# jhamrick/bayesian-quadrature

Hardware: NVIDIA B200
Metric: expected_Z_var candidate evals/sec (higher is better)
Workload: dtype f64

## Files before the change

bayesian_quadrature_b200/csrc/bq_score.cu:

```cuda
#include <cstdlib>

#include "bq_common.cuh"

namespace bqb {


constexpr int CHUNK_FRAGS_MAX = 256;
#ifndef BQB_REL_GK
#define BQB_REL_GK 4
#endif

__device__ __forceinline__ unsigned smem_u32(const void *p) { return (unsigned)__cvta_generic_to_shared(p); }
__device__ __forceinline__ void mbar_init(unsigned long long *bar, unsigned count) {
    asm volatile("mbarrier.init.shared::cta.b64 [%0], %1;" ::"r"(smem_u32(bar)), "r"(count) : "memory");
}
__device__ __forceinline__ void mbar_init_fence() { asm volatile("fence.mbarrier_init.release.cluster;" ::: "memory"); }
__device__ __forceinline__ void mbar_expect_tx(unsigned long long *bar, unsigned bytes) {
    asm volatile("mbarrier.arrive.expect_tx.shared::cta.b64 _, [%0], %1;" ::"r"(smem_u32(bar)), "r"(bytes) : "memory");
}
__device__ __forceinline__ void mbar_wait(unsigned long long *bar, unsigned parity) {
    asm volatile(
        "{\n"
        ".reg .pred p;\n"
        "MBAR_WAIT:\n"
        "mbarrier.try_wait.parity.shared::cta.b64 p, [%0], %1;\n"
        "@p bra MBAR_DONE;\n"
        "bra MBAR_WAIT;\n"
        "MBAR_DONE:\n"
        "}" ::"r"(smem_u32(bar)), "r"(parity) : "memory");
}
__device__ __forceinline__ void bulk_g2s(void *dst, const void *src, unsigned bytes, unsigned long long *bar) {
    asm volatile("cp.async.bulk.shared::cluster.global.mbarrier::complete_tx::bytes [%0], [%1], %2, [%3];" ::"r"(smem_u32(dst)),
                 "l"(src), "r"(bytes), "r"(smem_u32(bar)) : "memory");
}

constexpr int SCR_STRIDE = 40;
constexpr int SCR_DENSE = 4;

__device__ __forceinline__ void fetch_points(double *row, const double *__restrict__ xa, long long base, int na, int lane) {
    if (base + lane < na) {
        const unsigned d = (unsigned)__cvta_generic_to_shared(row + lane);
        asm volatile("cp.async.ca.shared.global [%0], [%1], 8;" ::"r"(d), "l"(xa + base + lane) : "memory");
    } else {
        row[lane] = 0.0;
    }
}

template <int KS, int NT, int WARPS, bool STREAM, int TABN>
struct ScoreSmem {
    static constexpr int NBC = KS / 2;
    static __host__ __device__ constexpr int operands(int ndb_max, int chunk_frags, int nb_res) {
        return STREAM ? 2 * chunk_frags * 32 + ndb_max * KS * 32 : 2 * tri_frags(nb_res) * 32 + ndb_max * 2 * nb_res * 32;
    }
    static __host__ __device__ constexpr int scr(int nrow) { return (SCR_DENSE + nrow) * SCR_STRIDE + 64; }
    static __host__ __device__ constexpr int doubles(int n_small, int ndb_max, int chunk_frags, int nb_res, int nrow) {
        return n_small + operands(ndb_max, chunk_frags, nb_res) + WARPS * scr(nrow);
    }
};

template <int THREADS>
__device__ __forceinline__ void stage(double *dst, const double *__restrict__ src, int count) {
    const double2 *s2 = reinterpret_cast<const double2 *>(src);
    double2 *d2 = reinterpret_cast<double2 *>(dst);
    for (int i = threadIdx.x; i < count / 2; i += THREADS) d2[i] = __ldg(s2 + i);
}

template <int KS> struct KMask { using type = unsigned; };
template <> struct KMask<40> { using type = unsigned long long; };
template <> struct KMask<64> { using type = unsigned long long; };

constexpr double CUT_ARG = 72.0;
static_assert(CUT_ARG == 72.0, "keep in step with ScoreArgs::cut_arg and include/bq_b200.h");

__device__ __forceinline__ int float_key(float f) {
    const int i = __float_as_int(f);
    return i >= 0 ? i : (i ^ 0x7fffffff);
}
__device__ __forceinline__ float key_float(int k) { return __int_as_float(k >= 0 ? k : (k ^ 0x7fffffff)); }

template <int KS>
__device__ __forceinline__ void gen_masks(double xv, bool valid, double cut_l, double cut_tl, int nsp, int lane,
                                          const double *s_xs, typename KMask<KS>::type &mask_l, typename KMask<KS>::type &mask_tl) {
    using mask_t = typename KMask<KS>::type;
    constexpr int NW = (KS + 7) / 8;
    const double xc = fmin(fmax(xv, -1e30), 1e30);
    const int klo = valid ? float_key(__double2float_rd(xc)) : 0x7fffffff;
    const int khi = valid ? float_key(__double2float_ru(xc)) : (int)0x80000000;
    const double xlo = (double)key_float(__reduce_min_sync(0xffffffffu, klo));
    const double xhi = (double)key_float(__reduce_max_sync(0xffffffffu, khi));
    if (!(xlo <= xhi)) { mask_l = 0; mask_tl = 0; return; }
    const double c = 0.5 * (xlo + xhi), hw = 0.5 * (xhi - xlo);
    double dk[NW];
    double dmin = INFINITY;
#pragma unroll
    for (int i = 0; i < NW; ++i) {
        const int k = 32 * i + lane;
        dk[i] = (k < nsp) ? fabs(s_xs[k] - c) : INFINITY;
        dmin = fmin(dmin, dk[i]);
    }
    const float dcf = __int_as_float(__reduce_min_sync(0xffffffffu, __float_as_int(__double2float_ru(fmin(dmin, 3e38)))));
    const double reach = (double)dcf + hw;
    const double r2_l = fma(reach, reach, cut_l), r2_tl = fma(reach, reach, cut_tl);
    mask_t ml = 0, mt = 0;
#pragma unroll
    for (int i = 0; i < NW; ++i) {
        const double t = fmax(dk[i] - hw, 0.0), t2 = t * t;
        const bool in = 32 * i + lane < nsp;
        unsigned bl = __ballot_sync(0xffffffffu, in && t2 <= r2_l), bt = __ballot_sync(0xffffffffu, in && t2 <= r2_tl);
        bl |= bl >> 1; bl |= bl >> 2; bl &= 0x11111111u;
        bl = (bl | (bl >> 3)) & 0x03030303u; bl = (bl | (bl >> 6)) & 0x000f000fu; bl = (bl | (bl >> 12)) & 0xffu;
        bt |= bt >> 1; bt |= bt >> 2; bt &= 0x11111111u;
        bt = (bt | (bt >> 3)) & 0x03030303u; bt = (bt | (bt >> 6)) & 0x000f000fu; bt = (bt | (bt >> 12)) & 0xffu;
        ml |= (mask_t)bl << (8 * i);
        mt |= (mask_t)bt << (8 * i);
    }
    mask_l = ml;
    mask_tl = mt;
}

template <int NT> __host__ __device__ constexpr int exp_group() { return NT == 1 ? 8 : 4; }
template <int KS, int NT, int TABN, bool TL, int GK = exp_group<NT>()>
__device__ __forceinline__ void gen_exps(double (&bf)[KS][NT], const double (&x)[NT], double C, int d2max_hi,
                                         typename KMask<KS>::type mask, int kq, const double *s_xs, const double *s_atl,
                                         const double *s_tab, double (&tm)[NT], int tol2_hi, int (&close)[NT], int nkv = KS) {
    using mask_t = typename KMask<KS>::type;
    int minhi[NT];
#pragma unroll
    for (int nt = 0; nt < NT; ++nt) minhi[nt] = 0x7fffffff;
#pragma unroll
    for (int g = 0; g < (KS + GK - 1) / GK; ++g) {
        if ((mask >> (GK * g)) & (((mask_t)1 << GK) - 1)) {
#pragma unroll
            for (int j = 0; j < GK; ++j) {
                const int ks = GK * g + j;
                if (ks < KS) {
                    const double xs = s_xs[4 * ks + kq];
#pragma unroll
                    for (int nt = 0; nt < NT; ++nt) {
                        const double d = x[nt] - xs;
                        const double d2 = d * d;
                        const double e = exp_kernel<TABN>(d2, C, d2max_hi, s_tab);
                        bf[ks][nt] = e;
                        if (TL) {
                            minhi[nt] = min(minhi[nt], __double2hiint(d2));
                            if (ks < nkv) tm[nt] = fma(s_atl[4 * ks + kq], e, tm[nt]);
                        }
                    }
                }
            }
        }
    }
    if (TL) {
#pragma unroll
        for (int nt = 0; nt < NT; ++nt) close[nt] = (minhi[nt] <= tol2_hi);
    }
}

__device__ __forceinline__ int isclose_exact(double x, const double *s_xs, const double *s_tol, int nsp, int kq) {
    int c = 0;
    for (int k = kq; k < nsp; k += 4) c |= (fabs(x - s_xs[k]) <= s_tol[k]);
    return c;
}

__device__ __forceinline__ void async_commit() { asm volatile("cp.async.commit_group;" ::: "memory"); }
template <int N> __device__ __forceinline__ void async_wait() { asm volatile("cp.async.wait_group %0;" ::"n"(N) : "memory"); }

template <int KS, int NT>
__device__ __forceinline__ void row_block_acc(const double *af, int lim, const double (&bf)[KS][NT], double (&c0)[NT],
                                              double (&c1)[NT], double (&e0)[NT], double (&e1)[NT],
                                              typename KMask<KS>::type mask) {
    using mask_t = typename KMask<KS>::type;
    constexpr bool DUAL = (NT == 1);
#pragma unroll
    for (int ks = 0; ks < KS; ks += 2) {
        if (ks >= lim) break;
        if (mask & ((mask_t)3 << ks)) {
            const double a0 = af[ks * 32], a1 = af[(ks + 1) * 32];
#pragma unroll
            for (int nt = 0; nt < NT; ++nt) {
                dmma(c0[nt], c1[nt], a0, bf[ks][nt]);
                if (DUAL) dmma(e0[nt], e1[nt], a1, bf[ks + 1][nt]);
                else dmma(c0[nt], c1[nt], a1, bf[ks + 1][nt]);
            }
        }
    }
}
template <int NT>
__device__ __forceinline__ void row_block_finish(const double (&c0)[NT], const double (&c1)[NT], const double (&e0)[NT],
                                                 const double (&e1)[NT], double (&q0)[NT], double (&q1)[NT]) {
    constexpr bool DUAL = (NT == 1);
#pragma unroll
    for (int nt = 0; nt < NT; ++nt) {
        const double r0 = DUAL ? c0[nt] + e0[nt] : c0[nt], r1 = DUAL ? c1[nt] + e1[nt] : c1[nt];
        q0[nt] = fma(r0, r0, q0[nt]);
        q1[nt] = fma(r1, r1, q1[nt]);
    }
}
template <int KS, int NT>
__device__ __forceinline__ void row_block(const double *af, int lim, const double (&bf)[KS][NT], double (&q0)[NT],
                                          double (&q1)[NT], typename KMask<KS>::type mask) {
    double c0[NT], c1[NT], e0[NT], e1[NT];
#pragma unroll
    for (int nt = 0; nt < NT; ++nt) { c0[nt] = c1[nt] = e0[nt] = e1[nt] = 0.0; }
    row_block_acc<KS, NT>(af, lim, bf, c0, c1, e0, e1, mask);
    row_block_finish<NT>(c0, c1, e0, e1, q0, q1);
}

template <int KS, int NT, int K0>
__device__ __forceinline__ void pair_group(const double *afA, const double *afB, int limA, const double (&bf)[KS][NT],
                                           double (&a0)[NT], double (&a1)[NT], double (&b0)[NT], double (&b1)[NT],
                                           double (&c0)[NT], double (&c1)[NT], double (&d0)[NT], double (&d1)[NT]) {
    constexpr int ks = K0;
    if (ks + 4 <= limA) {
        double fa[4], fb[4];
#pragma unroll
        for (int j = 0; j < 4; ++j) { fa[j] = afA[(ks + j) * 32]; fb[j] = afB[(ks + j) * 32]; }
#pragma unroll
        for (int j = 0; j < 4; j += 2)
#pragma unroll
            for (int nt = 0; nt < NT; ++nt) {
                dmma(a0[nt], a1[nt], fa[j], bf[ks + j][nt]);
                dmma(c0[nt], c1[nt], fb[j], bf[ks + j][nt]);
                dmma(b0[nt], b1[nt], fa[j + 1], bf[ks + j + 1][nt]);
                dmma(d0[nt], d1[nt], fb[j + 1], bf[ks + j + 1][nt]);
            }
    } else if (ks + 2 <= limA) {
        const double fa0 = afA[ks * 32], fa1 = afA[(ks + 1) * 32];
        double fb[4];
#pragma unroll
        for (int j = 0; j < 4; ++j) fb[j] = afB[(ks + j) * 32];
#pragma unroll
        for (int nt = 0; nt < NT; ++nt) {
            dmma(a0[nt], a1[nt], fa0, bf[ks][nt]);
            dmma(c0[nt], c1[nt], fb[0], bf[ks][nt]);
            dmma(b0[nt], b1[nt], fa1, bf[ks + 1][nt]);
            dmma(d0[nt], d1[nt], fb[1], bf[ks + 1][nt]);
            dmma(c0[nt], c1[nt], fb[2], bf[ks + 2][nt]);
            dmma(d0[nt], d1[nt], fb[3], bf[ks + 3][nt]);
        }
    } else {
        const double fb0 = afB[ks * 32], fb1 = afB[(ks + 1) * 32];
#pragma unroll
        for (int nt = 0; nt < NT; ++nt) {
            dmma(c0[nt], c1[nt], fb0, bf[ks][nt]);
            dmma(d0[nt], d1[nt], fb1, bf[ks + 1][nt]);
        }
    }
}

template <int KS, int NT, bool PLAIN = false>
__device__ __forceinline__ void row_block_pair(const double *afA, const double *afB, int limA, const double (&bf)[KS][NT],
                                               double (&q0)[NT], double (&q1)[NT], typename KMask<KS>::type mask, int g0, int kend) {
    using mask_t = typename KMask<KS>::type;
    static_assert(KS % 4 == 0 && KS <= 64, "k-steps come in groups of 4, at most 16 groups");
    double a0[NT], a1[NT], b0[NT], b1[NT], c0[NT], c1[NT], d0[NT], d1[NT];
#pragma unroll
    for (int nt = 0; nt < NT; ++nt) { a0[nt] = a1[nt] = b0[nt] = b1[nt] = c0[nt] = c1[nt] = d0[nt] = d1[nt] = 0.0; }
    const int kstop = min(kend, limA + 2);
#define BQB_GRP(G)                                                                                                       \
    case G:                                                                                                              \
        if constexpr (4 * (G) < KS) {                                                                                    \
            if (4 * (G) >= kstop) break;                                                                                 \
            if (mask & ((mask_t)15 << (4 * (G))))                            \
                pair_group<KS, NT, 4 * (G)>(afA, afB, limA, bf, a0, a1, b0, b1, c0, c1, d0, d1);                         \
        }                                                                                                                \
        [[fallthrough]];
#define BQB_GRP_PLAIN(G)                                                                                                 \
    if constexpr (4 * (G) < KS) {                                                                                        \
        if (4 * (G) < kstop) {                                                                                           \
            pair_group<KS, NT, 4 * (G)>(afA, afB, limA, bf, a0, a1, b0, b1, c0, c1, d0, d1);
// ... 187 lines not shown
__device__ __forceinline__ void tri_pass(const double *af_res, double (&bf)[KS][NT], double (&q0)[NT], double (&q1)[NT],
                                         int nb, int lane, typename KMask<KS>::type mask, int k0, const Wide<NT> &w) {
    using mask_t = typename KMask<KS>::type;
    static_assert(ROLLED || !REL, "the band-relative tile needs the rolled row-block loop");
    phase_sync<ALIGN>();
    if constexpr (ROLLED) {
        row_blocks_rolled<KS, NT, TABN, REL>(af_res + lane, 0, nb, bf, q0, q1, mask, k0, w);
    } else {
#pragma unroll
        for (int rb = 0; rb < KS / 2; ++rb) {
            constexpr int BITS = 8 * sizeof(mask_t);
            const mask_t low = (2 * rb + 2 >= BITS) ? ~(mask_t)0 : (((mask_t)1 << (2 * rb + 2)) - 1);
            if (rb < nb && (mask & low)) row_block<KS, NT>(af_res + tri_frags(rb) * 32 + lane, 2 * rb + 2, bf, q0, q1, mask);
        }
    }
}

struct SlabPlan {
    int klo, W, rb_first, R, nchunk;
};
template <int KS>
__device__ __forceinline__ SlabPlan make_slab_plan(typename KMask<KS>::type um, int nks, int nb, int cap_frags) {
    SlabPlan p;
    if (um == 0) { p.klo = p.W = p.rb_first = p.R = p.nchunk = 0; return p; }
    const unsigned long long m = um;
    const int lo = __ffsll((long long)m) - 1, hi = 64 - __clzll((long long)m);
    p.klo = lo & ~3;
    const int khi = min((hi + 3) & ~3, nks);
    p.W = khi - p.klo;
    p.rb_first = p.klo >> 1;
    p.R = max(2, (cap_frags / p.W) & ~1);
    p.nchunk = (nb - p.rb_first + p.R - 1) / p.R;
    return p;
}
struct Stream {
    unsigned long long *bar;
    double *buf;
    int stride;
    unsigned phase;
};
__device__ __forceinline__ void slab_issue(const double *__restrict__ op, const SlabPlan &p, int c, int nb, const Stream &st, int b,
                                           int lane) {
    const int rb0 = p.rb_first + c * p.R, n = min(nb - rb0, p.R);
    if (lane == 0) mbar_expect_tx(st.bar + b, (unsigned)(n * p.W * 256));
    __syncwarp();
    if (lane < n)
        bulk_g2s(st.buf + b * st.stride + lane * p.W * 32, op + (size_t)(tri_frags(rb0 + lane) + p.klo) * 32, (unsigned)(p.W * 256),
                 st.bar + b);
}
template <int KS, int NT, int TABN, bool REL>
__device__ __forceinline__ void slab_rows(const double *buf, const SlabPlan &p, int rb0, int rb1, double (&bf)[KS][NT],
                                          double (&q0)[NT], double (&q1)[NT], typename KMask<KS>::type mask, int lane, int k0,
                                          const Wide<NT> &w) {
    if constexpr (REL) {
        if (w.on) {
            const int kfirst = __ffsll((long long)w.mask) - 1;
#pragma unroll 1
            for (int rb = max(rb0, kfirst >> 1); rb < rb1; ++rb)
                wide_row_block<KS, NT, TABN>(buf + ((rb - rb0) * p.W - p.klo) * 32 + lane, 2 * rb + 2, w, bf, q0, q1);
            return;
        }
    }
    if (!mask) return;
    int g0, kend;
    mask_groups(mask, g0, kend);
    const int kfirst = k0 + __ffsll((long long)(unsigned long long)mask) - 1;
    int rb = rb0;
    const bool rect = REL && plain_band(mask, g0, kend);
    const int kend2 = (64 - __clzll((long long)(unsigned long long)mask) + 1) & ~1;
    const int rbf = rect ? min(rb1, max(rb0, ((k0 + kend2) >> 1) & ~1)) : rb1;
#pragma unroll 1
    for (; rb + 1 < rbf; rb += 2) {
        if (2 * rb + 4 <= kfirst) continue;
        const double *afA = buf + ((rb - rb0) * p.W - p.klo + k0) * 32 + lane;
        if (REL && rect) row_block_pair<KS, NT, REL>(afA, afA + p.W * 32, 2 * rb + 2 - k0, bf, q0, q1, mask, g0, kend);
        else row_block_pair<KS, NT>(afA, afA + p.W * 32, 2 * rb + 2 - k0, bf, q0, q1, mask, g0, kend);
    }
    if constexpr (REL) {
        if (rect && rb + 1 < rb1) {
            const int npair = (rb1 - rb) >> 1;
            rect_dispatch<KS, NT>(kend2 >> 1, buf + ((rb - rb0) * p.W - p.klo + k0) * 32 + lane, npair, p.W * 32, 2 * p.W * 32, 0, 0, bf, q0,
                                  q1);
            rb += 2 * npair;
        }
    }
    if (rb < rb1) row_block<KS, NT>(buf + ((rb - rb0) * p.W - p.klo + k0) * 32 + lane, 2 * rb + 2 - k0, bf, q0, q1, mask);
}
template <int KS, int NT, int TABN, bool REL>
__device__ __forceinline__ void slab_pass(const double *__restrict__ op, const SlabPlan &p, bool res, bool first_sub, Stream &st,
                                          double (&bf)[KS][NT], double (&q0)[NT], double (&q1)[NT], int nb, int lane, int warp,
                                          typename KMask<KS>::type mask, int k0, const Wide<NT> &w) {
    const int nch = res ? (p.nchunk ? 1 : 0) : p.nchunk;
    const int R = res ? nb - p.rb_first : p.R;
#pragma unroll 1
    for (int c = 0; c < nch; ++c) {
        const int b = res ? 0 : (c & 1);
        if (!res || first_sub) {
            mbar_wait(st.bar + b, (st.phase >> b) & 1u);
            st.phase ^= 1u << b;
        }
        const int rb0 = p.rb_first + c * R;
        slab_rows<KS, NT, TABN, REL>(st.buf + b * st.stride, p, rb0, min(nb, rb0 + R), bf, q0, q1, mask, lane, k0, w);
        if (!res) {
            __syncthreads();
            if (warp == 0 && c + 2 < nch) slab_issue(op, p, c + 2, nb, st, b, lane);
        }
    }
}

template <int KB, int NT, int GK = exp_group<NT>()>
__device__ __forceinline__ void dense_acc(const double *af, int nk, const double (&bf)[KB][NT], typename KMask<KB>::type mask,
                                          double (&c0)[NT], double (&c1)[NT], double (&e0)[NT], double (&e1)[NT]) {
    using mask_t = typename KMask<KB>::type;
#pragma unroll
    for (int g = 0; g < KB / GK; ++g) {
        if ((mask >> (GK * g)) & (((mask_t)1 << GK) - 1)) {
            double fa[GK];
#pragma unroll
            for (int j = 0; j < GK; ++j) fa[j] = (GK * g + j < nk) ? af[(GK * g + j) * 32] : 0.0;
#pragma unroll
            for (int j = 0; j < GK; j += 2)
#pragma unroll
                for (int nt = 0; nt < NT; ++nt) {
                    dmma(c0[nt], c1[nt], fa[j], bf[GK * g + j][nt]);
                    dmma(e0[nt], e1[nt], fa[j + 1], bf[GK * g + j + 1][nt]);
                }
        }
    }
}

template <int NT>
__device__ __forceinline__ void park_q(double (&q0)[NT], double (&q1)[NT], double *scr, int row, int col0, int kq, int pq) {
#pragma unroll
    for (int nt = 0; nt < NT; ++nt) {
#pragma unroll
        for (int o = 4; o < 32; o <<= 1) {
            q0[nt] += __shfl_xor_sync(0xffffffffu, q0[nt], o);
            q1[nt] += __shfl_xor_sync(0xffffffffu, q1[nt], o);
        }
        if (pq == 0) *reinterpret_cast<double2 *>(scr + row * SCR_STRIDE + col0 + nt * 8 + 2 * kq) = make_double2(q0[nt], q1[nt]);
    }
}

template <int KS, int NT, int WARPS, int MINB, bool STREAM, int TABN, int ALIGN, bool ROLLED, int BK, int MODE>
__global__ void __launch_bounds__(WARPS * 32, MINB) bq_score_kernel(ScoreArgs a) {
    constexpr bool EPI = MODE == 1, PRED = MODE == 2;
    constexpr bool REL = BK > 0;
    constexpr int KB = REL ? BK : KS;
    static_assert(!REL || (BK % 8 == 0 && BK <= KS), "band tile: whole exp groups, no larger than the class");
    using rmask_t = typename KMask<KB>::type;
    constexpr int GKK = REL ? BQB_REL_GK : exp_group<NT>();
    using SM = ScoreSmem<KS, NT, WARPS, STREAM, TABN>;
    constexpr bool LOCKSTEP = STREAM || ALIGN != 0;
    static_assert(ALIGN <= 1 || WARPS % ALIGN == 0, "barrier groups of whole warps");
    constexpr int THREADS = WARPS * 32;
    constexpr int SUB = 4 / NT;
    extern __shared__ __align__(16) double smem[];
    const Layout lay = a.lay;
    __shared__ __align__(16) double s_tab[TABN];
    double *s_small = smem;
    double *s_ops = s_small + lay.n_small;
    double *s_af_l = s_ops;
    constexpr bool RT_SIZES = KS > 16;
    const int nb_res = RT_SIZES ? a.nb_res : KS / 2, nrow_res = RT_SIZES ? a.nrow_res : 8 * a.ndb_max;
    double *s_af_d = STREAM ? s_ops + 2 * a.chunk_frags * 32 : s_af_l + tri_frags(nb_res) * 32;
    double *s_af_t = s_af_d + a.ndb_max * 2 * nb_res * 32;
    double *s_scr = s_ops + SM::operands(a.ndb_max, a.chunk_frags, nb_res);

    const int tid = threadIdx.x, lane = tid & 31, warp = tid >> 5;
    const int inst = a.inst0 + blockIdx.y;
    const double *M = a.models + (size_t)inst * lay.total;

    __shared__ int s_cta_st;
    if (tid == 0) s_cta_st = 0;
    for (int i = tid; i < TABN; i += THREADS) s_tab[i] = a.exp_tab[(TABN == 2048 ? 0 : 2048) + i];
    for (int i = tid; i < lay.n_small; i += THREADS) s_small[i] = M[i];
    __syncthreads();
    const int nc = (int)s_small[H_NC], nsp = (int)s_small[H_NSP], ndb = (int)s_small[H_NDB];
    const int nb = nsp >> 3, nks = nsp >> 2;
    __shared__ __align__(8) unsigned long long s_bar[2];
    __shared__ unsigned long long s_wm[STREAM ? 4 * WARPS : 1];
    int wm_set = 0;
    Stream strm{s_bar, s_ops, a.chunk_frags * 32, 0u};
    if constexpr (STREAM) {
        if (tid == 0) {
            mbar_init(s_bar, 1);
            mbar_init(s_bar + 1, 1);
            mbar_init_fence();
        }
    } else {
        stage<THREADS>(s_af_l, M + lay.off_af_l_tri, tri_frags(nb) * 32);
        stage<THREADS>(s_af_t, M + lay.off_af_tl_tri, tri_frags(nb) * 32);
    }
    stage<THREADS>(s_af_d, M + lay.off_af_l_dense, ndb * nks * 32);
    __syncthreads();

    const double *s_xs = s_small + lay.off_xs, *s_tol = s_small + lay.off_tol, *s_atl = s_small + lay.off_atl;
    const double nhl = s_small[H_NHL];
    const double Cl = nhl * ExpC<TABN>::INVN, Ctl = s_small[H_NHTL] * ExpC<TABN>::INVN;
    const int dmax_l = exp_d2max_hi(nhl), dmax_tl = exp_d2max_hi(s_small[H_NHTL]);
    using mask_t = typename KMask<KS>::type;
    const double cut_l = a.cut_arg / fabs(nhl), cut_tl = a.cut_arg / fabs(s_small[H_NHTL]);
    unsigned long long n_kstep = 0;
    const int tol2_hi = __double2hiint(s_small[H_TOL2MAX]) + 1;
    double *scr = s_scr + warp * SM::scr(nrow_res);

    const double *xa = a.x_a + (size_t)(inst / a.xa_group) * a.xa_stride;
    double *o_esm = a.esm ? a.esm + (size_t)inst * a.out_stride : nullptr;
    double *o_em = a.em ? a.em + (size_t)inst * a.out_stride : nullptr;
    int *o_st = a.status ? a.status + (size_t)inst * a.out_stride : nullptr;

    const int kq = lane & 3, pq = lane >> 2;
    constexpr int UNIT = 8 * NT * WARPS;
    const int n_units = (a.na + UNIT - 1) / UNIT;
    const int G = gridDim.x, cta = blockIdx.x;
    const int full = n_units / (G * SUB);
    const int R = n_units - full * G * SUB;
    const int r_lo = full * G * SUB + (int)(((long long)cta * R) / G);
    const int r_n = (int)(((long long)(cta + 1) * R) / G) - (int)(((long long)cta * R) / G);
    const int n_it = full + (r_n > 0 ? 1 : 0);
    auto tile_u = [&](int it) { return it < full ? (it * G + cta) * SUB : r_lo; };
    auto tile_n = [&](int it) { return it < full ? SUB : r_n; };
    double best_v = INFINITY;
    long long best_i = 0x7fffffffffffffffLL;

    int xb = 0;
    double *xrows = scr + (SCR_DENSE + nrow_res) * SCR_STRIDE;
    if (n_it > 0) fetch_points(xrows, xa, (long long)tile_u(0) * UNIT + warp * (8 * NT * tile_n(0)), a.na, lane);
    async_commit();

    for (int it = 0; it < n_it; ++it) {
        const int nsub = tile_n(it);
        const int npw = 8 * NT * nsub;
        const int base = tile_u(it) * UNIT + warp * npw;
        const double *xrow = xrows + 32 * xb;
        async_wait<0>();
        __syncwarp();
        xb ^= 1;
        if (it + 1 < n_it)
            fetch_points(xrows + 32 * xb, xa, (long long)tile_u(it + 1) * UNIT + warp * (8 * NT * tile_n(it + 1)), a.na, lane);
        async_commit();
        if (!LOCKSTEP && base >= a.na) continue;

        mask_t wmask_l, wmask_tl;
        {
            const double xv = xrow[lane];
            gen_masks<KS>(xv, lane < npw && base + lane < a.na && isfinite(xv), cut_l, cut_tl, nsp, lane, s_xs, wmask_l, wmask_tl);
        }
        SlabPlan plan_l, plan_tl;
        bool res_l = false, res_tl = false;
        if constexpr (STREAM) {
            unsigned long long *wm = s_wm + wm_set * 2 * WARPS;
            wm_set ^= 1;
            if (lane == 0) { wm[2 * warp] = wmask_l; wm[2 * warp + 1] = wmask_tl; }
            __syncthreads();
            unsigned long long um_l = 0, um_tl = 0;
#pragma unroll
            for (int w = 0; w < WARPS; ++w) { um_l |= wm[2 * w]; um_tl |= wm[2 * w + 1]; }
            plan_l = make_slab_plan<KS>((mask_t)um_l, nks, nb, a.chunk_frags);
            plan_tl = make_slab_plan<KS>((mask_t)um_tl, nks, nb, a.chunk_frags);
            res_l = (nb - plan_l.rb_first) * plan_l.W <= 2 * a.chunk_frags;
            res_tl = (nb - plan_tl.rb_first) * plan_tl.W <= 2 * a.chunk_frags;
        }

        int k0_l = 0, k0_tl = 0;
        Wide<NT> wd_l, wd_tl;
        wd_l.on = wd_tl.on = false;
        if constexpr (REL) {
            auto band = [&](mask_t m, int &k0, Wide<NT> &w, double C, int dmax) {
                w.mask = m; w.C = C; w.dmax = dmax; w.kq = lane & 3; w.s_xs = s_xs; w.s_tab = s_tab;
                w.kbeg = w.kend = 0;
                if (!m) return;
                const int lo = __ffsll((long long)(unsigned long long)m) - 1, hi = 64 - __clzll((long long)(unsigned long long)m);
                w.kbeg = lo & ~7; w.kend = hi;
                const unsigned long long mb = (unsigned long long)m >> lo;
                w.on = (hi - (lo & ~1) > KB) || (mb & (mb + 1)) != 0 || a.force_wide;
                k0 = w.on ? 0 : (lo & ~1);
            };
            band(wmask_l, k0_l, wd_l, Cl, dmax_l);
            band(wmask_tl, k0_tl, wd_tl, Ctl, dmax_tl);
        }

        constexpr int NPH = STREAM ? 2 : 1;
#pragma unroll
        for (int ph = 0; ph < NPH; ++ph) {
            const bool do_l = !STREAM || ph == 0, do_tl = !STREAM || ph == 1;
            const SlabPlan &plan = ph ? plan_tl : plan_l;
            const bool res = ph ? res_tl : res_l;
            const double *op = M + (ph ? lay.off_af_tl_tri : lay.off_af_l_tri);
            if constexpr (STREAM) {
                if (ph == 1) __syncthreads();
                if (res && plan.nchunk && warp == 0) {
                    const int n = nb - plan.rb_first;
                    if (lane == 0) mbar_expect_tx(strm.bar, (unsigned)(n * plan.W * 256));
                    __syncwarp();
                    if (lane < n)
                        bulk_g2s(strm.buf + lane * plan.W * 32, op + (size_t)(tri_frags(plan.rb_first + lane) + plan.klo) * 32,
                                 (unsigned)(plan.W * 256), strm.bar);
                }
            }
#pragma unroll 1
            for (int sub = 0; sub < nsub; ++sub) {
                const int col0 = sub * 8 * NT;
                double x[NT];
#pragma unroll
                for (int nt = 0; nt < NT; ++nt) {
                    const double v = xrow[col0 + nt * 8 + pq];
                    x[nt] = isfinite(v) ? v : 0.0;
                }
                double bf[KB][NT];
                double q0[NT], q1[NT], tm[NT];
                int close[NT];
#pragma unroll
                for (int nt = 0; nt < NT; ++nt) { q0[nt] = q1[nt] = tm[nt] = 0.0; close[nt] = 0; }
                mask_t mask = wmask_l;
                const mask_t mask_tl = wmask_tl;
                if constexpr (REL) {
#pragma unroll
                    for (int nt = 0; nt < NT; ++nt) wd_l.x[nt] = wd_tl.x[nt] = x[nt];
                }
                if constexpr (STREAM) {
                    if (!res && plan.nchunk && warp == 0) {
                        slab_issue(op, plan, 0, nb, strm, 0, lane);
                        if (plan.nchunk > 1) slab_issue(op, plan, 1, nb, strm, 1, lane);
                    }
                }

                if (do_l) {
                    phase_sync<ALIGN>();
                    const rmask_t rm_l = REL ? (wd_l.on ? (rmask_t)0 : (rmask_t)(mask >> k0_l)) : (rmask_t)mask;
                    gen_exps<KB, NT, TABN, false, GKK>(bf, x, Cl, dmax_l, rm_l, kq, s_xs + 4 * k0_l, s_atl, s_tab, tm, tol2_hi, close);
                    if constexpr (STREAM)
                        slab_pass<KB, NT, TABN, REL>(op, plan, res, sub == 0, strm, bf, q0, q1, nb, lane, warp, rm_l, k0_l, wd_l);
                    else tri_pass<KB, NT, TABN, ALIGN, ROLLED, REL>(s_af_l, bf, q0, q1, nb, lane, rm_l, k0_l, wd_l);
                    if (a.work) n_kstep += count_ksteps<KS>(mask, nb) + ndb * __popcll((unsigned long long)mask);
#pragma unroll
                    for (int db = 0; db < 3; ++db) {
                        if (db < ndb) {
                            const double *af = s_af_d + (db * nks) * 32 + lane;
                            double c0[NT], c1[NT], e0[NT], e1[NT];
#pragma unroll
                            for (int nt = 0; nt < NT; ++nt) { c0[nt] = c1[nt] = e0[nt] = e1[nt] = 0.0; }
                            if (REL && wd_l.on) {
#pragma unroll 1
                                for (int kw = wd_l.kbeg; kw < wd_l.kend; kw += KB) {
                                    const rmask_t rw = window_mask<KB>(wd_l.mask, kw);
                                    if (!rw) continue;
                                    gen_exps<KB, NT, TABN, false>(bf, x, Cl, dmax_l, rw, kq, s_xs + 4 * kw, s_atl, s_tab, tm, tol2_hi, close);
                                    dense_acc<KB, NT>(af + kw * 32, nks - kw, bf, rw, c0, c1, e0, e1);
                                }
                            } else {
                                dense_acc<KB, NT, GKK>(af + k0_l * 32, nks - k0_l, bf, rm_l, c0, c1, e0, e1);
                            }
                            if (!RT_SIZES || db * 8 + pq < nrow_res) {
#pragma unroll
                                for (int nt = 0; nt < NT; ++nt)
                                    *reinterpret_cast<double2 *>(scr + (SCR_DENSE + db * 8 + pq) * SCR_STRIDE + col0 + nt * 8 + 2 * kq) =
                                        make_double2(c0[nt] + e0[nt], c1[nt] + e1[nt]);
                            }
                        }
                    }
                    park_q<NT>(q0, q1, scr, 0, col0, kq, pq);
                }

                if (do_tl) {
#pragma unroll
                    for (int nt = 0; nt < NT; ++nt) { q0[nt] = q1[nt] = 0.0; }
                    phase_sync<ALIGN>();
                    mask = mask_tl;
                    const rmask_t rm_tl = REL ? (wd_tl.on ? (rmask_t)0 : (rmask_t)(mask >> k0_tl)) : (rmask_t)mask;
                    if (REL && wd_tl.on) {
#pragma unroll 1
                        for (int kw = wd_tl.kbeg; kw < wd_tl.kend; kw += KB) {
                            const rmask_t rw = window_mask<KB>(wd_tl.mask, kw);
                            if (!rw) continue;
                            int cw[NT];
                            gen_exps<KB, NT, TABN, true>(bf, x, Ctl, dmax_tl, rw, kq, s_xs + 4 * kw, s_atl + 4 * kw, s_tab, tm, tol2_hi, cw,
                                                         KS - kw);
#pragma unroll
                            for (int nt = 0; nt < NT; ++nt) close[nt] |= cw[nt];
                        }
                    } else {
                        gen_exps<KB, NT, TABN, true, GKK>(bf, x, Ctl, dmax_tl, rm_tl, kq, s_xs + 4 * k0_tl, s_atl + 4 * k0_tl, s_tab, tm,
                                                          tol2_hi, close, KS - k0_tl);
                    }
#pragma unroll
                    for (int nt = 0; nt < NT; ++nt)
                        if (close[nt]) close[nt] = isclose_exact(x[nt], s_xs, s_tol, nsp, kq);
                    if constexpr (STREAM)
                        slab_pass<KB, NT, TABN, REL>(op, plan, res, sub == 0, strm, bf, q0, q1, nb, lane, warp, rm_tl, k0_tl, wd_tl);
                    else tri_pass<KB, NT, TABN, ALIGN, ROLLED, REL>(s_af_t, bf, q0, q1, nb, lane, rm_tl, k0_tl, wd_tl);
                    if (a.work) n_kstep += count_ksteps<KS>(mask, nb);
                    park_q<NT>(q0, q1, scr, 1, col0, kq, pq);
#pragma unroll
                    for (int nt = 0; nt < NT; ++nt) {
                        tm[nt] += __shfl_xor_sync(0xffffffffu, tm[nt], 1);
                        tm[nt] += __shfl_xor_sync(0xffffffffu, tm[nt], 2);
                        close[nt] |= __shfl_xor_sync(0xffffffffu, close[nt], 1);
                        close[nt] |= __shfl_xor_sync(0xffffffffu, close[nt], 2);
                        if (kq == 0) {
                            scr[2 * SCR_STRIDE + col0 + nt * 8 + pq] = tm[nt];
                            scr[3 * SCR_STRIDE + col0 + nt * 8 + pq] = close[nt] ? 1.0 : 0.0;
                        }
                    }
                }
            }
        }
        __syncwarp();

        const int p = base + lane;
        if (lane < npw && p < a.na) {
            const double xv = xrow[lane];
            const double Zm = s_small[H_ZM];
            double esm, em;
            int st = ST_OK;
            if (!isfinite(xv)) {
                esm = em = nan("");
                st = ST_XA_BAD;
            } else if (!PRED && scr[3 * SCR_STRIDE + lane] != 0.0) {
                em = Zm; esm = Zm * Zm; st = ST_SHORTCUT;
            } else {
                const double qs = scr[lane], qt = scr[SCR_STRIDE + lane], tmv = scr[2 * SCR_STRIDE + lane];
                double *dr = scr + SCR_DENSE * SCR_STRIDE + lane;
                const double c_l = s_small[H_CL], thresh = s_small[H_THRESH];
                const double *s_xc = s_small + lay.off_xc;
                unsigned mask = 0;
                for (int j = 0; j < nc; ++j) {
                    const double dc = s_xc[j] - xv;
                    if (!PRED && fabs(dc) < thresh) mask |= 1u << j;
                    dr[j * SCR_STRIDE] = fma(c_l, exp_kernel<TABN>(dc * dc, Cl, dmax_l, s_tab), dr[j * SCR_STRIDE]);
                }
                double qc = 0, vg = 0, va = 0, bg = 0, kaa;
                bool pd = true;
                if (mask == 0) {
                    const double *Lc = s_small + lay.off_lcc0, *ug = s_small + lay.off_ug0, *ua = s_small + lay.off_ua0,
                                 *rd = s_small + lay.off_rd0;
                    for (int i = 0; i < nc; ++i) {
                        double s = dr[i * SCR_STRIDE];
                        for (int k = 0; k < i; ++k) s = fma(-Lc[i * NC_MAX + k], dr[k * SCR_STRIDE], s);
                        s *= rd[i];
                        dr[i * SCR_STRIDE] = s;
                        qc = fma(s, s, qc); vg = fma(s, ug[i], vg); va = fma(s, ua[i], va);
                        bg = fma(ug[i], ua[i], bg);
                    }
                    kaa = s_small[H_KAA_E];
                } else {
                    const double *S0 = s_small + lay.off_s0, *wb = s_small + lay.off_wb, *wa = s_small + lay.off_wa;
                    const double j1 = s_small[H_J1];
                    double Lc[NC_MAX * (NC_MAX + 1) / 2], ug[NC_MAX], ua[NC_MAX];
                    for (int i = 0; i < nc && pd; ++i) {
                        for (int j = 0; j <= i; ++j) {
                            double s = S0[i * NC_MAX + j];
                            if (i == j && ((mask >> i) & 1u)) s += j1;
                            for (int k = 0; k < j; ++k) s -= Lc[i * (i + 1) / 2 + k] * Lc[j * (j + 1) / 2 + k];
                            if (i == j) {
                                if (!(s > 0.0)) { pd = false; break; }
                                Lc[i * (i + 1) / 2 + i] = sqrt(s);
                            } else {
                                Lc[i * (i + 1) / 2 + j] = s / Lc[j * (j + 1) / 2 + j];
                            }
                        }
                    }
                    if (pd) {
                        for (int i = 0; i < nc; ++i) {
                            double s = dr[i * SCR_STRIDE], sg = wb[i], sa = wa[i];
                            for (int k = 0; k < i; ++k) {
                                const double l = Lc[i * (i + 1) / 2 + k];
                                s -= l * dr[k * SCR_STRIDE]; sg -= l * ug[k]; sa -= l * ua[k];
                            }
                            const double d = Lc[i * (i + 1) / 2 + i];
                            s /= d; sg /= d; sa /= d;
                            dr[i * SCR_STRIDE] = s; ug[i] = sg; ua[i] = sa;
                            qc = fma(s, s, qc); vg = fma(s, sg, vg); va = fma(s, sa, va);
                            bg = fma(sg, sa, bg);
                        }
                    }
                    kaa = s_small[H_KAA_N];
                }
                const double s_ = kaa - (qs + qc);
                if (PRED) {
                    esm = dr[(nc + 1) * SCR_STRIDE] + va;
                    em = s_small[H_KTT] - qt;
                } else if (!pd || !(s_ > 0.0)) {
                    em = Zm; esm = Zm * Zm; st = ST_NOTPD;
                } else {
                    const double ba = s_small[H_BA_S] + bg;
                    const double kg = dr[nc * SCR_STRIDE] + vg;
                    const double ka = dr[(nc + 1) * SCR_STRIDE] + va;
                    const double diff = xv - s_small[H_MU];
                    const double b_a = s_small[H_CB] * exp_tab<TABN>((diff * diff) * s_small[H_NHB], s_tab);
                    const double A_a = (b_a - kg) / s_;
                    const double A_sc_l = ba - A_a * ka;
                    const double tC = s_small[H_KTT] - qt;
                    const double a1 = tmv + 0.5 * tC;
                    const double a2 = 2.0 * tmv + 2.0 * tC;
                    if (a1 > MAX_EXPONENT) {
                        esm = em = INFINITY;
                    } else {
                        const double e1 = exp_tab<TABN>(a1, s_tab);
                        em = A_sc_l + A_a * e1;
                        if (a2 > MAX_EXPONENT) {
                            esm = INFINITY;
                        } else {
                            const double e2 = exp_tab<TABN>(a2, s_tab);
                            esm = (A_sc_l * A_sc_l) + (2 * A_sc_l * A_a * e1) + ((A_a * A_a) * e2);
                        }
                    }
                    if (isnan(esm) || esm < 0) st |= ST_ESM_BAD;
                    if (isnan(em)) st |= ST_EM_BAD;
                    if (isinf(esm)) st |= ST_ESM_INF;
                    if (isinf(em)) st |= ST_EM_INF;
                }
            }
            const int po = a.perm ? a.perm[p] : p;
            if (o_esm) o_esm[po] = esm;
            if (EPI) {
                const double evv = __dsub_rn(__dadd_rn(__dmul_rn(Zm, Zm), s_small[H_ZV]), esm);
                a.ev[po] = evv;
                if (evv < best_v || (evv == best_v && po < best_i)) { best_v = evv; best_i = po; }
            }
            if (o_em) o_em[po] = em;
            if (o_st) o_st[po] = st;
            if (st) {
                if (a.flags) atomicOr(a.flags + inst, st);
                if (a.cta_flags) atomicOr(&s_cta_st, st);
            }
        }
        __syncwarp();
    }
    if (a.work && lane == 0 && n_kstep) atomicAdd(a.work, n_kstep * NT);
    if (a.cta_flags) {
        __syncthreads();
        if (tid == 0) a.cta_flags[blockIdx.y * gridDim.x + blockIdx.x] = s_cta_st;
    }
    if (EPI) {
#pragma unroll
        for (int o = 16; o > 0; o >>= 1) {
            const double v2 = __shfl_xor_sync(0xffffffffu, best_v, o);
            const long long i2 = __shfl_xor_sync(0xffffffffu, best_i, o);
            if (v2 < best_v || (v2 == best_v && i2 < best_i)) { best_v = v2; best_i = i2; }
        }
        __syncthreads();
        double *rv = s_scr;
        long long *ri = reinterpret_cast<long long *>(s_scr + WARPS);
        if (lane == 0) { rv[warp] = best_v; ri[warp] = best_i; }
// ... 158 lines not shown
```

Baseline: 3.390 billion.

## Skip K_tl triangular pass for tiles provably far from all data points

For the 16-k-step non-stream, non-predict variant, each CTA computes the Frobenius norm of the staged K_tl triangular factor. From it, it derives a squared-distance threshold beyond which the K_tl contribution falls below roughly 2^-59 relative to ktt. Each warp then bounds the distance from its point tile's hull to the nearest data point, and tags the tile's tl mask with a high bit when it lies beyond that threshold. Tagged tiles run the triangular pass with an empty mask, saving DMMA work on far-away query tiles. The cost is an extra warp reduction per tile, a CTA-level norm computation, and a numerical approximation that depends on the error bound being valid.

Measured after the change: 3.452 billion (median of 6 runs). +1.8%, better.

```diff
diff --git a/bayesian_quadrature_b200/csrc/bq_score.cu b/bayesian_quadrature_b200/csrc/bq_score.cu
--- a/bayesian_quadrature_b200/csrc/bq_score.cu
+++ b/bayesian_quadrature_b200/csrc/bq_score.cu
@@ -116,6 +116,26 @@
     }
     mask_l = ml;
     mask_tl = mt;
+}
+
+template <int KS>
+__device__ __forceinline__ double hull_dist_lo(double xv, bool valid, int nsp, int lane, const double *s_xs) {
+    constexpr int NW = (KS + 7) / 8;
+    const double xc = fmin(fmax(xv, -1e30), 1e30);
+    const int klo = valid ? float_key(__double2float_rd(xc)) : 0x7fffffff;
+    const int khi = valid ? float_key(__double2float_ru(xc)) : (int)0x80000000;
+    const double xlo = (double)key_float(__reduce_min_sync(0xffffffffu, klo));
+    const double xhi = (double)key_float(__reduce_max_sync(0xffffffffu, khi));
+    if (!(xlo <= xhi)) return -1.0;
+    const double c = 0.5 * (xlo + xhi), hw = 0.5 * (xhi - xlo);
+    double dmin = INFINITY;
+#pragma unroll
+    for (int i = 0; i < NW; ++i) {
+        const int k = 32 * i + lane;
+        if (k < nsp) dmin = fmin(dmin, fabs(s_xs[k] - c));
+    }
+    const float dlf = __int_as_float(__reduce_min_sync(0xffffffffu, __float_as_int(__double2float_rd(fmin(dmin, 3e38)))));
+    return fmax((double)dlf - hw, 0.0);
 }
 
 template <int NT> __host__ __device__ constexpr int exp_group() { return NT == 1 ? 8 : 4; }
@@ -609,6 +629,7 @@
     constexpr int GKK = REL ? BQB_REL_GK : exp_group<NT>();
     using SM = ScoreSmem<KS, NT, WARPS, STREAM, TABN>;
     constexpr bool LOCKSTEP = STREAM || ALIGN != 0;
+    constexpr bool FAR = KS == 16 && MODE != 2 && !STREAM;
     static_assert(ALIGN <= 1 || WARPS % ALIGN == 0, "barrier groups of whole warps");
     constexpr int THREADS = WARPS * 32;
     constexpr int SUB = 4 / NT;
@@ -638,6 +659,8 @@
     __shared__ __align__(8) unsigned long long s_bar[2];
     __shared__ unsigned long long s_wm[STREAM ? 4 * WARPS : 1];
     int wm_set = 0;
+    if constexpr (FAR)
+        if (tid == 0) reinterpret_cast<double *>(s_wm)[0] = 0.0;
     Stream strm{s_bar, s_ops, a.chunk_frags * 32, 0u};
     if constexpr (STREAM) {
         if (tid == 0) {
@@ -651,6 +674,19 @@
     }
     stage<THREADS>(s_af_d, M + lay.off_af_l_dense, ndb * nks * 32);
     __syncthreads();
+    if constexpr (FAR) {
+        double f = 0.0;
+        for (int i = tid; i < tri_frags(nb) * 32; i += THREADS) f = fma(s_af_t[i], s_af_t[i], f);
+        f = warp_sum(f);
+        if (lane == 0) atomicAdd(reinterpret_cast<double *>(s_wm), f);
+        __syncthreads();
+        const double fa = reinterpret_cast<const double *>(s_wm)[0] * 1.000001;
+        const double lim = 0x1p-59 * s_small[H_KTT] / (fa * nsp);
+        __syncthreads();
+        if (tid == 0)
+            reinterpret_cast<double *>(s_wm)[0] = lim >= 1.0 ? 0.0 : lim > 1e-290 ? log(lim) / (2.0 * s_small[H_NHTL]) : INFINITY;
+        __syncthreads();
+    }
 
     const double *s_xs = s_small + lay.off_xs, *s_tol = s_small + lay.off_tol, *s_atl = s_small + lay.off_atl;
     const double nhl = s_small[H_NHL];
@@ -703,6 +739,10 @@
         {
             const double xv = xrow[lane];
             gen_masks<KS>(xv, lane < npw && base + lane < a.na && isfinite(xv), cut_l, cut_tl, nsp, lane, s_xs, wmask_l, wmask_tl);
+            if constexpr (FAR) {
+                const double dlo = hull_dist_lo<KS>(xv, lane < npw && base + lane < a.na && isfinite(xv), nsp, lane, s_xs);
+                if (dlo >= 0.0 && dlo * dlo * (1.0 - 1e-9) >= reinterpret_cast<const double *>(s_wm)[0]) wmask_tl |= 1u << 31;
+            }
         }
         SlabPlan plan_l, plan_tl;
         bool res_l = false, res_tl = false;
@@ -846,8 +886,12 @@
                         if (close[nt]) close[nt] = isclose_exact(x[nt], s_xs, s_tol, nsp, kq);
                     if constexpr (STREAM)
                         slab_pass<KB, NT, TABN, REL>(op, plan, res, sub == 0, strm, bf, q0, q1, nb, lane, warp, rm_tl, k0_tl, wd_tl);
-                    else tri_pass<KB, NT, TABN, ALIGN, ROLLED, REL>(s_af_t, bf, q0, q1, nb, lane, rm_tl, k0_tl, wd_tl);
-                    if (a.work) n_kstep += count_ksteps<KS>(mask, nb);
+                    else if constexpr (FAR) {
+                        const mask_t mt = (mask >> 31) ? (mask_t)0 : mask;
+                        tri_pass<KB, NT, TABN, ALIGN, ROLLED, REL>(s_af_t, bf, q0, q1, nb, lane, (rmask_t)mt, k0_tl, wd_tl);
+                        if (a.work) n_kstep += count_ksteps<KS>(mt, nb);
+                    } else tri_pass<KB, NT, TABN, ALIGN, ROLLED, REL>(s_af_t, bf, q0, q1, nb, lane, rm_tl, k0_tl, wd_tl);
+                    if (!FAR && a.work) n_kstep += count_ksteps<KS>(mask, nb);
                     park_q<NT>(q0, q1, scr, 1, col0, kq, pq);
 #pragma unroll
                     for (int nt = 0; nt < NT; ++nt) {
diff --git a/bench_micro/count_two_sided.py b/bench_micro/count_two_sided.py
--- /dev/null
+++ b/bench_micro/count_two_sided.py
@@ -0,0 +1,77 @@
+import argparse
+import json
+import os
+import sys
+
+import numpy as np
+
+sys.path.insert(0, os.path.dirname(os.path.dirname(os.path.abspath(__file__))))
+
+CUT_ARG = 72.0
+
+
+def masks(xa, x_s, w, nks):
+    tiles = xa[: xa.size // 32 * 32].reshape(-1, 32)
+    lo, hi = tiles.min(axis=1), tiles.max(axis=1)
+    c, hw = 0.5 * (lo + hi), 0.5 * (hi - lo)
+    d = np.abs(x_s[None, :] - c[:, None])
+    reach = d.min(axis=1) + hw
+    cut = CUT_ARG * 2.0 * w * w
+    t = np.maximum(d - hw[:, None], 0.0)
+    rel = t * t <= (reach * reach + cut)[:, None]
+    obs = np.zeros((rel.shape[0], 4 * nks), dtype=bool)
+    obs[:, : x_s.size] = rel
+    ks = obs.reshape(rel.shape[0], nks, 4).any(axis=2)
+    return (ks * (1 << np.arange(nks))).sum(axis=1).astype(np.int64)
+
+
+def count(m, nb):
+    m = (m | (m >> 1)) & 0x5555555555555555
+    m = m | (m << 1)
+    n = np.zeros_like(m)
+    for rb in range(nb):
+        low = m & ((1 << (2 * rb + 2)) - 1)
+        n += np.array([bin(int(v)).count("1") for v in low])
+    return n
+
+
+def reverse(m, nks):
+    return np.array([int(format(int(v), "0%db" % nks)[::-1], 2) for v in m], dtype=np.int64)
+
+
+def main():
+    ap = argparse.ArgumentParser()
+    ap.add_argument("--points", type=int, default=10 ** 6)
+    ap.add_argument("--t-l", type=int, default=0, help="reverse K_l columns below this k-step are not resident")
+    ap.add_argument("--t-tl", type=int, default=0, help="the same for K_tl")
+    args = ap.parse_args()
+    from bayesian_quadrature_b200 import synthetic
+    ns, nc = 64, 4
+    nsp, nks, nb = 64, 16, 8
+    x_s, _ = synthetic.observations(ns)
+    x_s = np.sort(x_s)
+    xa = synthetic.query_grid(ns, args.points)
+    out = {"points": args.points, "T_l": args.t_l, "T_tl": args.t_tl}
+    dmma_one = dmma_two = 0
+    for name, w, T in (("K_l", synthetic.PARAMS_L[1], args.t_l), ("K_tl", synthetic.PARAMS_TL[1], args.t_tl)):
+        m = masks(xa, x_s, w, nks)
+        r = reverse(m, nks)
+        low = (1 << T) - 1
+        f_cost, r_cost = count(m, nb), count(r, nb)
+        side = np.where(((r & low) == 0) & (r_cost < f_cost), 1, 0)
+        two = np.where(side == 1, r_cost, f_cost)
+        left = xa[: xa.size // 32 * 32].reshape(-1, 32).max(axis=1) < x_s[0]
+        right = xa[: xa.size // 32 * 32].reshape(-1, 32).min(axis=1) > x_s[-1]
+        out[name] = {"forward_per_tile": float(f_cost.mean()), "two_sided_per_tile": float(two.mean()),
+                     "cheaper_side_per_tile": float(np.minimum(f_cost, r_cost).mean()),
+                     "left_of_data_forward": float(f_cost[left].mean()), "right_of_data_forward": float(f_cost[right].mean()),
+                     "tiles_forward_reverse": [int((side == s).sum()) for s in range(2)]}
+        dense = ((nc + 2 + 7) // 8) * np.array([bin(int(v)).count("1") for v in m]) if name == "K_l" else 0
+        dmma_one += int((4 * (f_cost + dense)).sum())
+        dmma_two += int((4 * (two + dense)).sum())
+    out["predicted_executed_dmma_per_launch"] = {"forward_only": dmma_one, "two_sided": dmma_two, "ratio": dmma_two / dmma_one}
+    print(json.dumps(out, indent=1))
+
+
+if __name__ == "__main__":
+    main()
```
